# unum-cloud/usearch

Measured on AMD Instinct MI355X. Metric: QPS at recall@10>=0.95, 10000000x768 f16 cos, batch=10000, higher is better.
Workload: dtype f16

## Files before the change

usearch_amd/csrc/engine.hip:

```cpp
#include "engine.hpp"

#include <algorithm>
#include <atomic>
#include <chrono>
#include <cstdio>
#include <cstdlib>
#include <cstring>
#include <thread>

#include <hipcub/hipcub.hpp>

#include "casts.hpp"
#include "host_util.hpp"
#include "kernels.hpp"
#include "search_plan.hpp"

namespace usearch_amd {

static hipError_t scratch_malloc(void** out, std::size_t bytes) {
#ifdef USEARCH_AMD_EXPERIMENT_SCRATCH_MEMORY
    const std::size_t kind = env_size("USEARCH_AMD_SCRATCH_MEMORY", 0);
    if (kind == 1 || kind == 2) {
        const hipError_t e = hipExtMallocWithFlags(out, bytes, kind == 1 ? hipDeviceMallocUncached : hipDeviceMallocFinegrained);
        if (e == hipSuccess)
// ... 870 lines not shown
        ++call.passes;
        UA_HIP(hipStreamSynchronize(stream));
    }
    return nullptr;
}

const char* snapshot_t::search_finish(search_call_t& call, search_stats_t* stats) {
    if (stats)
        *stats = search_stats_t{};
    if (!call.workspace)
        return nullptr;
    struct hand_back_t {
        snapshot_t& owner;
        search_call_t& call;
        ~hand_back_t() {
            if (!call.keep_workspace)
                owner.give_back(call.workspace);
            call.workspace = nullptr;
        }
    } hand_back{*this, call};
    workspace_t& ws = *call.workspace;
    hipStream_t stream = call.stream;
    UA_HIP(hipSetDevice(device_));
    if (call.done) {
        UA_HIP(hipStreamSynchronize(stream));
        return nullptr;
    }

    const std::uint32_t first_grid = call.params.grid, first_lds = call.params.lds_bytes;
    const int first_mode = call.params.mode;
    for (int rung = 0;; ++rung) {
        UA_HIP(hipMemcpyAsync(ws.h_status, ws.d_queue, 24, hipMemcpyDeviceToHost, stream));
        UA_HIP(hipStreamSynchronize(stream));
        if (call.args.sketch_counters) {
            std::uint64_t counters[2];
            std::memcpy(counters, ws.h_status + 2, 16);
            call.plan.stats.sketch_tested += counters[0], call.plan.stats.sketch_pruned += counters[1];
        }
        if (call.params.mode == scratch_global_k) {
            if (ws.h_status[1])
                return "Search scratch overflow in the global-memory pass";
            break;
        }
        if (!ws.h_status[1])
            break;
        UA_HIP(hipMemcpyAsync(ws.h_status + 16, ws.d_status, call.count * 4, hipMemcpyDeviceToHost, stream));
        UA_HIP(hipStreamSynchronize(stream));
        std::vector<std::uint32_t> again;
        if (call.have_todo) {
            for (std::uint32_t q : call.todo)
                if (ws.h_status[16 + q] == status_overflow_k)
                    again.push_back(q);
        } else {
            for (std::uint32_t q = 0; q < call.count; ++q)
                if (ws.h_status[16 + q] == status_overflow_k)
                    again.push_back(q);
        }
        call.todo.swap(again);
        call.have_todo = true;
        call.reran = true;
        if (call.todo.empty())
            break;
        if (rung == 0)
            call.plan.stats.retried_lds = (std::uint32_t)call.todo.size();
        escalate(call.shape, call.knobs, call.plan, rung);
        if (call.plan.mode != scratch_global_k)
            UA_HIP(hipMemcpyAsync(ws.d_todo, call.todo.data(), call.todo.size() * 4, hipMemcpyHostToDevice, stream));
        if (const char* e = run_ladder(call))
            return e;
    }

    if (call.want_phases) {
        unsigned long long ticks[16] = {0};
        UA_HIP(hipMemcpy(ticks, call.args.phases, 128, hipMemcpyDeviceToHost));
        double total = 0;
        for (int i = 0; i < 6; ++i)
            total += (double)ticks[i];
        std::fprintf(stderr, "[usearch_amd] phases ef=%u grid=%u: setup %.1f%% pop+list %.1f%% visited %.1f%% distances %.1f%% "
                             "commit %.1f%% [heap push %.1f%% top insert %.1f%%, %llu candidates rechecked] dump %.1f%% (%.3g ticks); "
                             "frontier pushes %llu, lists ready ahead %llu\n",
                     call.plan.ef, first_grid, 100 * ticks[0] / total, 100 * ticks[1] / total, 100 * ticks[2] / total,
                     100 * ticks[3] / total, 100 * ticks[4] / total, 100 * ticks[8] / total, 100 * ticks[9] / total, ticks[10],
                     100 * ticks[5] / total, total, ticks[6], ticks[7]);
        if (ticks[15])
            std::fprintf(stderr, "[usearch_amd] a team's helpers: %llu hops, ticks measuring per hop %.0f %.0f %.0f %.0f\n", ticks[15],
                         (double)ticks[11] / (double)ticks[15], (double)ticks[12] / (double)ticks[15],
                         (double)ticks[13] / (double)ticks[15], (double)ticks[14] / (double)ticks[15]);
    }
    if (call.want_clock && ws.d_wave_clock && first_grid) {
        std::vector<unsigned long long> clock((std::size_t)first_grid * 2);
        UA_HIP(hipMemcpy(clock.data(), ws.d_wave_clock, clock.size() * 8, hipMemcpyDeviceToHost));
        unsigned long long first = ~0ull, last = 0;
        for (std::uint32_t w = 0; w < first_grid; ++w)
            first = std::min(first, clock[2 * w]), last = std::max(last, clock[2 * w + 1]);
        double gone = 0;
        for (std::uint32_t w = 0; w < first_grid; ++w)
            gone += (double)(clock[2 * w] - first) + (double)(last - clock[2 * w + 1]);
        const double span = (double)(last - first);
        call.plan.stats.tail_idle = span > 0 ? (float)(gone / (span * first_grid)) : 0.f;
        call.plan.stats.span_ms = (float)(span / 1e5);
        if (env_size("USEARCH_AMD_WAVE_CLOCK", 0) > 1) {
            unsigned long long bins[10] = {0};
            for (std::uint32_t w = 0; w < first_grid; ++w)
                ++bins[std::min<std::size_t>(9, (std::size_t)(10.0 * (double)(clock[2 * w + 1] - first) / std::max(span, 1.0)))];
            std::fprintf(stderr, "[usearch_amd] wave exits by tenth of the %.3f ms span (grid %u):", call.plan.stats.span_ms, first_grid);
            for (unsigned long long b : bins)
                std::fprintf(stderr, " %llu", b);
            std::fprintf(stderr, "; idle share %.4f\n", call.plan.stats.tail_idle);
        }
    }
    call.plan.stats.passes = call.passes;
    call.plan.stats.kernel_ms = call.total_ms;
    call.plan.stats.mode = (std::uint32_t)first_mode + 1;
    call.plan.stats.grid = first_grid;
    call.plan.stats.lds_bytes = first_lds;
    if (stats)
        *stats = call.plan.stats;
    if (call.sketch_auto && call.count >= 1024)
        judge_sketch(call.plan.stats.sketch_tested, call.plan.stats.sketch_pruned);
    return nullptr;
}

const char* snapshot_t::search_device(const void* queries, std::size_t count, std::size_t stride_bytes,
                                      std::size_t wanted, std::size_t expansion, std::uint64_t* keys,
                                      float* distances, std::uint64_t* counts, std::uint64_t* visited,
                                      std::uint64_t* computed, hipStream_t stream, const search_tuning_t& tuning,
                                      search_stats_t* stats, bool timed, const search_extras_t* extras) {
    if (stats)
        *stats = search_stats_t{};
    search_call_t call;
    const char* error = search_begin(call, queries, count, stride_bytes, wanted, expansion, keys, distances, counts, visited,
                                     computed, stream, tuning, timed, extras);
    if (error) {
        if (call.workspace)
            give_back(call.workspace);
        return error;
    }
    return search_finish(call, stats);
}

const char* snapshot_t::tune(const void* queries, std::size_t count, std::size_t stride_bytes, std::size_t wanted, std::size_t expansion,
                             std::uint32_t max_trials, std::uint32_t* trials_made) {
    if (trials_made)
        *trials_made = 0;
    max_trials = std::min<std::uint32_t>(max_trials, (std::uint32_t)placement_max_draws_k);
    if (!count || !wanted || !max_trials || !d_vectors_)
        return nullptr;
    UA_HIP(hipSetDevice(device_));
    struct block_t {
        void* p = nullptr;
        ~block_t() { (void)hipFree(p); }
    } results;
    const std::size_t pad = 256, keys_bytes = (count * wanted * 8 + pad - 1) / pad * pad, distances_bytes = (count * wanted * 4 + pad - 1) / pad * pad,
                      column = (count * 8 + pad - 1) / pad * pad;
    UA_HIP(hipMalloc(&results.p, keys_bytes + distances_bytes + 3 * column));
    std::uint8_t* base = static_cast<std::uint8_t*>(results.p);
    const std::uint32_t before = placement_.draws;
    {
        std::lock_guard<std::mutex> lock(pool_mutex_);
        tuning_trials_ = max_trials;
        placement_trials_left_ = max_trials, placement_losses_ = 0, placement_reopens_ = 2;
    }
    const char* failure = nullptr;
    for (std::uint32_t launch = 0; launch < max_trials + 1u && !failure; ++launch) {
        failure = search_device(queries, count, stride_bytes, wanted, expansion, reinterpret_cast<std::uint64_t*>(base),
                                reinterpret_cast<float*>(base + keys_bytes), reinterpret_cast<std::uint64_t*>(base + keys_bytes + distances_bytes),
// ... 436 lines not shown
```

usearch_amd/csrc/kernels.hpp:

```cpp
#pragma once
#include <type_traits>
#include <hip/hip_runtime.h>

#include "common.hpp"
#include "sketch.hpp"

namespace usearch_amd {

#define UA_DEVICE __device__ __forceinline__


UA_DEVICE std::uint32_t lane_id() { return threadIdx.x & 63u; }

template <bool global_ak> UA_DEVICE void wave_sync() {
    if constexpr (global_ak) {
        __builtin_amdgcn_fence(__ATOMIC_RELEASE, "workgroup");
        __builtin_amdgcn_wave_barrier();
        __builtin_amdgcn_fence(__ATOMIC_ACQUIRE, "workgroup");
    } else {
        __builtin_amdgcn_fence(__ATOMIC_RELEASE, "workgroup", "local");
        __builtin_amdgcn_wave_barrier();
        __builtin_amdgcn_fence(__ATOMIC_ACQUIRE, "workgroup", "local");
    }
}
// ... 949 lines not shown
    return chunks * ((scalar_ak == scalar_f16_k || scalar_ak == scalar_bf16_k) ? 32u : 16u);
}

struct team_t {
    std::uint32_t count;
    std::uint32_t leader_in;
    std::uint32_t reserved[2];
    query_norm_t a2;
};
static_assert(sizeof(team_t) <= 64, "the engine reserves 64 bytes for the control block");
constexpr std::uint32_t team_exit_k = 0xFFFFFFFFu;
constexpr std::uint32_t team_ahead_rows_k = 32;
constexpr std::uint32_t team_block_bytes_k = 64 + team_ahead_rows_k * 4;
UA_DEVICE std::uint32_t* team_ahead_list(team_t* team) {
    return reinterpret_cast<std::uint32_t*>(reinterpret_cast<std::uint8_t*>(team) + 64);
}

struct team_landing_t {
    std::uint32_t cell[3] = {0, 0, 0};
};
UA_DEVICE void team_touch_rows(const snapshot_view_t& ix, const std::uint32_t* ahead, std::uint32_t helper, team_landing_t& landing) {
    const std::uint32_t lane = lane_id();
    const std::uint32_t row = helper * 8 + (lane >> 3);
    const std::uint32_t slot = row < team_ahead_rows_k ? ahead[row] : none_slot_k;
    const std::uint32_t halves = (ix.bytes_per_vector + 63u) / 64u;
    const std::uint8_t* half = ix.vectors + (std::uint64_t)slot * ix.row_stride + (lane & 7u) * 64u;
    if (slot != none_slot_k && (lane & 7u) < halves)
        asm volatile("global_load_dword %0, %1, off" : "=&v"(landing.cell[0]) : "v"(half) : "memory");
    if (slot != none_slot_k && 8u + (lane & 7u) < halves)
        asm volatile("global_load_dword %0, %1, off" : "=&v"(landing.cell[1]) : "v"(half + 512) : "memory");
    if (slot != none_slot_k && 16u + (lane & 7u) < halves)
        asm volatile("global_load_dword %0, %1, off" : "=&v"(landing.cell[2]) : "v"(half + 1024) : "memory");
}
UA_DEVICE void team_landing_alive(const team_landing_t& landing) {
    asm volatile("" ::"v"(landing.cell[0]), "v"(landing.cell[1]), "v"(landing.cell[2]));
}

constexpr int team_waves_k = 5;

UA_DEVICE void team_barrier() { asm volatile("s_waitcnt lgkmcnt(0)\n\ts_barrier" ::: "memory"); }

template <int metric_ak, int scalar_ak, int lanes_ak, int loads_ak>
UA_DEVICE void team_share(const snapshot_view_t& ix, const std::uint8_t* query_lds, query_norm_t a2, const std::uint32_t* slots,
                          float* out, std::uint32_t count, std::uint32_t part, std::uint32_t parts, bool in_turn = false) {
    const std::uint32_t per_part = in_turn ? 64u / lanes_ak : (count + parts - 1) / parts;
    const std::uint32_t begin = part * per_part;
    const std::uint32_t end = (in_turn && part + 1 == parts) || begin + per_part > count ? count : begin + per_part;
    if (begin < end)
        measure_rows<metric_ak, scalar_ak, lanes_ak, loads_ak, false, 1>(ix, query_lds, a2, slots + begin, out + begin, end - begin);
}

template <int metric_ak, int scalar_ak, int lanes_ak, int unroll_ak, int mode_ak, int epl_ak, int frontier_ak, int team_ak = 1,
          bool plain_ak = false>
UA_DEVICE bool search_one(const snapshot_view_t& ix, const search_args_t& args, std::uint32_t q,
                          std::uint8_t* query_lds, std::uint8_t* heaps, std::uint32_t* visits, team_t* team = nullptr) {
    constexpr bool global_ak = mode_ak == scratch_global_k;
    constexpr bool in_top_ak = frontier_ak == frontier_top_k;
    static_assert(!in_top_ak || (epl_ak > 0 && !global_ak), "the frontier rides in the register layout of `top`");
    static_assert(!plain_ak || (lanes_ak <= 2 && mode_ak == scratch_hash_k && team_ak == 1 && !in_top_ak), "short rows over the global hash");
    using mem = scratch_gt<global_ak>;
    const std::uint32_t lane = lane_id();
    const std::uint32_t ef = args.ef, wanted = args.wanted;
    const scratch_layout_t layout = scratch_layout(epl_ak ? 0 : ef, in_top_ak ? 0 : args.next_cap, 0);
    top_gt<epl_ak, global_ak, in_top_ak> top;
    top.reset(reinterpret_cast<cand_t*>(heaps + layout.top));
    cand_t* next = reinterpret_cast<cand_t*>(heaps + layout.next);
    std::uint32_t* cand_slots = reinterpret_cast<std::uint32_t*>(heaps + layout.cand_slots);
    float* cand_distances = reinterpret_cast<float*>(heaps + layout.cand_distances);
    const std::uint32_t visits_mask = global_ak ? 0u : args.hash_cap - 1;
    const std::uint32_t visits_limit = global_ak ? 0xFFFFFFFFu : args.hash_cap - args.hash_cap / 4;

#ifdef USEARCH_AMD_PHASES
    std::uint64_t phase_mark = args.phases ? __builtin_amdgcn_s_memtime() : 0;
    std::uint64_t phase_ticks[6] = {0, 0, 0, 0, 0, 0};
    std::uint32_t diagnostic_pushes = 0, diagnostic_ready = 0, diagnostic_rechecks = 0;
    std::uint64_t diagnostic_push_ticks = 0, diagnostic_insert_ticks = 0;
    auto tick = [&](int phase) {
        if (args.phases) {
            const std::uint64_t now = __builtin_amdgcn_s_memtime();
            phase_ticks[phase] += now - phase_mark;
            phase_mark = now;
        }
    };
#else
    auto tick = [](int) {};
#endif
    const std::uint64_t query_row = !plain_ak && args.query_ids ? args.query_ids[q] : q;
    const query_norm_t a2 = stage_query<metric_ak, scalar_ak, lanes_ak>(
        ix, args.queries + query_row * args.query_stride, query_lds);

    if constexpr (!global_ak) {
        uint4* cells = reinterpret_cast<uint4*>(visits);
        const uint4 empty = {none_slot_k, none_slot_k, none_slot_k, none_slot_k};
        for (std::uint32_t i = lane; i < args.hash_cap / 4; i += 64)
            cells[i] = empty;
#ifdef USEARCH_AMD_EXPERIMENT_NO_SLAB_CLEAR_WAIT
        wave_sync<false>();
#else
        if constexpr (mode_ak == scratch_hash_k)
            wave_sync<true>();
        else
            wave_sync<false>();
#endif
    }

    constexpr bool seen_ak = lanes_ak <= 2 && mode_ak == scratch_hash_k && team_ak == 1;
#ifdef USEARCH_AMD_EXPERIMENT_NO_ASIDE
    constexpr bool aside_ak = false;
#else
    constexpr bool aside_ak = plain_ak && lanes_ak == 2;
#endif
    std::uint32_t* seen = nullptr;
    std::uint32_t seen_mask = 0;
    std::uint32_t* aside = nullptr;
    std::uint32_t aside_mask = 0, aside_count = 0;
    if constexpr (aside_ak) {
        aside = reinterpret_cast<std::uint32_t*>(query_lds + args.aside_offset);
        aside_mask = args.aside_cells - 1;
        for (std::uint32_t i = lane; i < args.aside_cells; i += 64)
            aside[i] = none_slot_k;
        wave_sync<false>();
    }
    if constexpr (seen_ak) {
        if (args.seen_cells) {
            seen = reinterpret_cast<std::uint32_t*>(query_lds + args.seen_offset);
            seen_mask = args.seen_cells - 1;
            for (std::uint32_t i = lane; i < args.seen_cells; i += 64)
                seen[i] = none_slot_k;
            wave_sync<false>();
        }
        if (!plain_ak && args.probe_mode == probe_plain_k) {
            std::uint32_t* claim = reinterpret_cast<std::uint32_t*>(query_lds + args.claim_offset);
            for (std::uint32_t i = lane; i < args.claim_bits / 32; i += 64)
                claim[i] = 0u;
            wave_sync<false>();
        }
    }

    constexpr bool sketch_ak = metric_ak == metric_cos_k && f32_math<scalar_ak>() && lanes_ak == 8 && team_ak == 1 && !global_ak && !plain_ak &&
                               unroll_ak % 100 == 12;
    bool sketch_on = false;
    float sketch_margin = 0.f;
    std::uint32_t sketch_tested = 0, sketch_pruned = 0;
    if constexpr (sketch_ak) {
        if (ix.sketch && args.sketch_counters) {
            const float* a = reinterpret_cast<const float*>(query_lds);
            const float* column = ix.sketch_directions + lane;
            float sums[4] = {0.f, 0.f, 0.f, 0.f};
            std::uint32_t i = 0;
            for (; i + 16 <= ix.dimensions; i += 16) {
                float d[16];
#pragma unroll
                for (int u = 0; u < 16; ++u)
                    d[u] = column[(std::size_t)(i + u) * sketch_columns_k];
#pragma unroll
                for (int u = 0; u < 16; ++u)
                    sums[u & 3] = __builtin_fmaf(a[i + u], d[u], sums[u & 3]);
            }
            for (; i < ix.dimensions; ++i)
                sums[0] = __builtin_fmaf(a[i], column[(std::size_t)i * sketch_columns_k], sums[0]);
            const float projected = (sums[0] + sums[1]) + (sums[2] + sums[3]);
            sketch_on = uniform_u32(sketch_norm_in_range((double)a2.f) ? 1u : 0u) != 0u;
            reinterpret_cast<float*>(query_lds + args.sketch_offset)[lane] = sketch_on ? projected / __builtin_sqrtf(a2.f) : 0.f;
            sketch_margin = sketch_slack(ix.dimensions);
            wave_sync<false>();
        }
    }

    std::uint32_t computed = 0, cycles = 0;
    constexpr int loads_ak = unroll_ak % 100, rows_ak = unroll_ak / 100 + 1;
    auto measure = [&](std::uint32_t count) {
        measure_rows<metric_ak, scalar_ak, lanes_ak, loads_ak, global_ak, 1>(ix, query_lds, a2, cand_slots, cand_distances,
                                                                            count);
        computed += count;
    };
    auto measure_hop = [&](std::uint32_t count, float radius_now) {
        if constexpr (sketch_ak) {
            if (sketch_on && top.size == ef) {
                const std::uint32_t sub = lane & 7u, group = lane >> 3;
                const float* coefficients = reinterpret_cast<const float*>(query_lds + args.sketch_offset) + sub * 8;
                const float4 q0 = *reinterpret_cast<const float4*>(coefficients), q1 = *reinterpret_cast<const float4*>(coefficients + 4);
                const std::uint32_t my_slot = lane < count ? mem::load(cand_slots + lane) : 0u;
                for (std::uint32_t base = 0; base < count; base += 32) {
                    uint4 record[4];
#pragma unroll
                    for (int r = 0; r < 4; ++r) {
                        const std::uint32_t ci = base + (std::uint32_t)r * 8 + group;
                        record[r] = uint4{0u, 0u, 0u, 0u};
                        if (ci < count)
                            record[r] = *reinterpret_cast<const uint4*>(ix.sketch + (std::uint64_t)mem::load(cand_slots + ci) * sketch_record_bytes_k + sub * 16);
                    }
#pragma unroll
                    for (int r = 0; r < 4; ++r) {
                        const std::uint32_t ci = base + (std::uint32_t)r * 8 + group;
                        const uint4 v = record[r];
                        const std::uint32_t last = sub == 7u ? 0u : v.w;
                        float dot = 0.f;
                        dot = __builtin_fmaf(half_bits_to_float(v.x & 0xFFFFu), q0.x, dot);
                        dot = __builtin_fmaf(half_bits_to_float(v.x >> 16), q0.y, dot);
                        dot = __builtin_fmaf(half_bits_to_float(v.y & 0xFFFFu), q0.z, dot);
                        dot = __builtin_fmaf(half_bits_to_float(v.y >> 16), q0.w, dot);
                        dot = __builtin_fmaf(half_bits_to_float(v.z & 0xFFFFu), q1.x, dot);
                        dot = __builtin_fmaf(half_bits_to_float(v.z >> 16), q1.y, dot);
                        dot = __builtin_fmaf(half_bits_to_float(last & 0xFFFFu), q1.z, dot);
                        dot = __builtin_fmaf(half_bits_to_float(last >> 16), q1.w, dot);
                        float residual = sub == 7u ? __builtin_bit_cast(float, v.w) : 0.f;
#pragma unroll
                        for (int offset = 1; offset < 8; offset <<= 1) {
                            dot += xor_lane(dot, offset);
                            residual += xor_lane(residual, offset);
                        }
                        if (sub == 0u && ci < count)
                            mem::store(cand_distances + ci, sketch_lower_bound(dot, residual, sketch_margin));
                    }
                }
                wave_sync<false>();
                const float bound = lane < count ? mem::load(cand_distances + lane) : 0.f;
                const std::uint64_t survivors = ballot(lane < count && !(bound >= radius_now));
                const std::uint32_t kept = popcount64(survivors);
                sketch_tested += count, sketch_pruned += count - kept;
                if (kept < count) {
                    const bool survivor = lane_bit(survivors);
                    const std::uint32_t rank = rank_below(survivors, lane);
                    wave_sync<false>();
                    if (survivor)
                        mem::store(cand_slots + rank, my_slot);
                    wave_sync<false>();
                    if (kept)
                        measure_rows<metric_ak, scalar_ak, lanes_ak, loads_ak, global_ak, rows_ak>(ix, query_lds, a2, cand_slots, cand_distances, kept);
                    const float mine = survivor ? mem::load(cand_distances + rank) : bound;
                    wave_sync<false>();
                    if (lane < count) {
                        mem::store(cand_slots + lane, my_slot);
                        mem::store(cand_distances + lane, mine);
                    }
                    wave_sync<false>();
                    computed += count;
                    return;
                }
            }
        }
        if constexpr (team_ak > 1) {
            if (lane == 0)
                team->count = count, team->leader_in = 1u, team->a2 = a2;
            team_barrier();
            team_share<metric_ak, scalar_ak, lanes_ak, loads_ak>(ix, query_lds, a2, cand_slots, cand_distances, count, 0, 4);
            team_barrier();
        } else {
            measure_rows<metric_ak, scalar_ak, lanes_ak, loads_ak, global_ak, rows_ak>(ix, query_lds, a2, cand_slots,
                                                                                       cand_distances, count);
        }
        computed += count;
    };
    auto allowed = [&](std::uint32_t slot) -> bool {
        if constexpr (plain_ak)
            return true;
        if (!ix.has_tombstones && !args.allow_bits && !args.exclude_own)
            return true;
        bool ok = !(args.exclude_own && slot == (std::uint32_t)query_row);
        if (ok && ix.has_tombstones)
            ok = ix.keys[slot] != free_key_k;
        if (ok && args.allow_bits) {
            const std::uint32_t word = slot >> 5, bit = 1u << (slot & 31);
            if (args.known_bits && !(args.known_bits[word] & bit)) {
                ok = slot * 0x9E3779B1u <= args.guess_threshold;
                if (lane == 0) {
                    const std::uint32_t at = atomicAdd(args.ask_cursor, 1u);
                    if (at < args.ask_cap)
                        args.ask_slots[at] = slot, args.ask_keys[at] = ix.keys[slot];
                }
            } else {
                ok = (args.allow_bits[word] & bit) != 0;
            }
        }
        return uniform_u32(ok ? 1u : 0u) != 0;
    };

    std::uint32_t closest = ix.entry_slot;
    if (lane == 0)
        mem::store(cand_slots, closest);
    wave_sync<global_ak>();
    measure(1);
    float closest_distance = uniform_f32(mem::load(cand_distances));
    const std::uint32_t beam_level = plain_ak ? 0u : args.beam_level;
    for (std::uint32_t level = ix.max_level; level > beam_level; --level) {
        bool changed;
        do {
            changed = false;
            const std::uint32_t* list = ix.upper + (std::uint64_t)(ix.upper_ref[closest] + (level - 1)) * ix.m;
            for (std::uint32_t tile = 0; tile < ix.m; tile += 64) {
                const std::uint32_t cell = tile + lane;
                const std::uint32_t neighbor = cell < ix.m ? list[cell] : none_slot_k;
                const std::uint32_t count = popcount64(ballot(neighbor != none_slot_k));
                if (!count)
                    break;
                if (lane < count)
                    mem::store(cand_slots + lane, neighbor);
                wave_sync<global_ak>();
                measure(count);
                const float mine = lane < count ? mem::load(cand_distances + lane) : __builtin_inff();
                float best = mine;
#pragma unroll
                for (int offset = 32; offset >= 1; offset >>= 1)
                    best = fminf(best, __shfl_xor(best, offset, 64));
                if (best < closest_distance) {
                    const std::uint32_t winner =
                        (std::uint32_t)__ffsll((long long)ballot(lane < count && mine == best)) - 1;
                    closest_distance = best;
                    closest = read_lane_u32(neighbor, winner);
                    changed = true;
                }
                wave_sync<global_ak>();
            }
            ++cycles;
        } while (changed);
    }

    std::uint32_t next_size = 0, visits_count = 0, peak_next = 1;
    bool overflow = false;
    if (lane == 0)
        mem::store(cand_slots, closest);
    wave_sync<global_ak>();
    measure(1);
    float radius = uniform_f32(mem::load(cand_distances));
// ... 174 lines not shown
                }
                tick(3);
            }
        }
    }
    for (; !pipelined;) {
        std::uint32_t expanded;
        if constexpr (in_top_ak) {
            float open_distance;
            std::uint32_t owner_lane, owner_cell;
            if (!top.first_open(open_distance, expanded, owner_lane, owner_cell))
                break;
            top.close(owner_lane, owner_cell);
        } else {
            if (!next_size)
                break;
            const cand_t candidate = mem::load(next);
            const float candidate_distance = -uniform_f32(cand_distance(candidate));
            if (candidate_distance > radius && top.size == ef)
                break;
            expanded = uniform_u32(cand_slot(candidate));
        }
        ++cycles;
        const std::uint32_t* list = list_of(expanded);
        const bool list_ready = expanded == ahead_slot;
#ifdef USEARCH_AMD_PHASES
        diagnostic_ready += list_ready ? 1u : 0u;
#endif
        const std::uint32_t ready_cell = ahead_cell;
        std::uint32_t first_cell = none_slot_k;
        if (!list_ready && lane < cells)
            first_cell = list[lane];
        uint4 inline_row = {0u, 0u, 0u, 0u};
        if constexpr (inline_ak) {
            if (inline_rows) {
                if (list_ready)
                    inline_row = ahead_row;
                else if (lane < cells)
                    inline_row = reinterpret_cast<const uint4*>(ix.nbr0_rows)[(std::uint64_t)expanded * cells + lane];
            }
        }
        bool popped = false;
        auto pop_now = [&]() {
            popped = true;
            ahead_slot = none_slot_k;
            if constexpr (in_top_ak) {
                float ahead_distance;
                std::uint32_t ahead_lane, ahead_index;
                if (!top.first_open(ahead_distance, ahead_slot, ahead_lane, ahead_index))
                    ahead_slot = none_slot_k;
            } else {
                heap_pop<global_ak>(next, next_size);
                if (next_size)
                    ahead_slot = uniform_u32(cand_slot(mem::load(next)));
            }
            if (ahead_slot != none_slot_k) {
                ahead_cell = lane < cells ? list_of(ahead_slot)[lane] : none_slot_k;
                if constexpr (inline_ak)
                    if (inline_rows && lane < cells)
                        ahead_row = reinterpret_cast<const uint4*>(ix.nbr0_rows)[(std::uint64_t)ahead_slot * cells + lane];
            }
        };
        if (in_top_ak || !list_ready || cells > 64 || mode_ak == scratch_global_k)
            pop_now();
        for (std::uint32_t tile = 0; tile < cells; tile += 64) {
            const std::uint32_t cell = tile + lane;
            const std::uint32_t neighbor =
                tile == 0 ? (list_ready ? ready_cell : first_cell) : (cell < cells ? list[cell] : none_slot_k);
            const bool present = neighbor != none_slot_k;
            const std::uint32_t present_count = popcount64(ballot(present));
            if (!present_count)
                break;
            if (visits_count + present_count > visits_limit ||
                (!in_top_ak && next_size - (popped ? 0u : 1u) + present_count > args.next_cap)) {
                overflow = true;
                break;
            }
            tick(1);
            bool fresh;
            float early_mine = 0.f;
            bool early_done = false;
            std::uint64_t asked_mask = 0;
            bool measured_early = false;
            if constexpr (mode_ak == scratch_global_k) {
                fresh = visits_set<mode_ak>(visits, visits_mask, neighbor, present);
            } else {
                std::uint32_t h = hash_slot(neighbor) & visits_mask;
                std::uint32_t old = neighbor;
                bool asks = present;
                std::uint32_t seen_cell = 0;
                if constexpr (seen_ak) {
                    if (seen) {
                        seen_cell = ((neighbor * 0x9E3779B1u) >> 9) & seen_mask;
                        asks = present && seen[seen_cell] != neighbor;
                    }
                }
                bool shadow_done = false;
                auto shadow_work = [&]() {
                    if (shadow_done)
                        return;
                    shadow_done = true;
                if constexpr (inline_ak) {
                    if (inline_rows) {
                        partial_t p;
                        accumulate_chunk<metric_ak, scalar_ak>(p, query_lds, 0, inline_row);
                        early_mine = finalize_distance<metric_ak, scalar_ak>(p, a2, ix.dimensions);
                        early_done = true;
                    }
                }
                if constexpr (early_ak) {
                    if (early_rows && tile == 0) {
                        asked_mask = ballot(asks);
                        const std::uint32_t asked = popcount64(asked_mask);
                        if (asks)
                            cand_slots[rank_below(asked_mask, lane)] = neighbor;
                        wave_sync<false>();
                        if (asked)
                            measure_rows<metric_ak, scalar_ak, lanes_ak, loads_ak, false, 1>(ix, query_lds, a2, cand_slots, cand_distances, asked);
                        measured_early = true;
                    }
                }
                };
                std::uint32_t probe_mode = probe_swap_k;
#ifdef USEARCH_AMD_EXPERIMENT_PROBE_MODES
                if constexpr (seen_ak)
                    probe_mode = args.probe_mode;
#endif
                const bool load_first = probe_mode == probe_load_first_k;
                if (probe_mode == probe_plain_k) {
                    std::uint32_t* claim = reinterpret_cast<std::uint32_t*>(query_lds + args.claim_offset);
                    const std::uint32_t claim_mask = args.claim_bits - 1;
                    bool looking = asks;
                    for (;;) {
                        std::uint32_t cell_value = none_slot_k;
                        if (looking)
                            cell_value = __hip_atomic_load(visits + h, __ATOMIC_RELAXED, __HIP_MEMORY_SCOPE_AGENT);
                        if (!popped)
                            pop_now();
                        shadow_work();
                        const bool wants = looking && cell_value == none_slot_k;
                        if (looking && cell_value == neighbor)
                            looking = false;
                        if (ballot(wants)) {
                            const std::uint32_t bit = h & claim_mask;
                            bool won = false;
                            if (wants) {
                                const std::uint32_t before = __hip_atomic_fetch_or(claim + (bit >> 5), 1u << (bit & 31u), __ATOMIC_RELAXED,
                                                                                   __HIP_MEMORY_SCOPE_WORKGROUP);
                                won = ((before >> (bit & 31u)) & 1u) == 0u;
                                claim[bit >> 5] = 0u;
                            }
                            if (won) {
                                __hip_atomic_store(visits + h, neighbor, __ATOMIC_RELAXED, __HIP_MEMORY_SCOPE_AGENT);
                                old = none_slot_k, looking = false;
                            }
                        }
                        if (looking && !wants)
                            h = (h + 1) & visits_mask;
                        if (!ballot(looking))
                            break;
                    }
                } else {
                if (asks) {
                    if (load_first) {
                        old = __hip_atomic_load(visits + h, __ATOMIC_RELAXED, __HIP_MEMORY_SCOPE_AGENT);
                        if (old == none_slot_k)
                            old = atomicCAS(visits + h, none_slot_k, neighbor);
                    } else {
                        old = atomicCAS(visits + h, none_slot_k, neighbor);
                    }
                }
                if (!popped)
                    pop_now();
                shadow_work();
                if constexpr (aside_ak) {
                    bool taken = asks && old != none_slot_k && old != neighbor;
                    const std::uint64_t taken_mask = ballot(taken);
                    if (taken_mask) {
                        if (aside_count + popcount64(taken_mask) > aside_mask - aside_mask / 4) {
                            overflow = true;
                            break;
                        }
                        std::uint32_t cell = ((neighbor * 0x9E3779B1u) >> 11) & aside_mask;
                        do {
                            std::uint32_t there = neighbor;
                            if (taken)
                                there = atomicCAS(aside + cell, none_slot_k, neighbor);
                            if (taken && (there == none_slot_k || there == neighbor))
                                old = there, taken = false;
                            cell = (cell + 1) & aside_mask;
                        } while (ballot(taken));
                        aside_count += popcount64(ballot(lane_bit(taken_mask) && old == none_slot_k));
                    }
                }
                while (!aside_ak && old != none_slot_k && old != neighbor) {
                    h = (h + 1) & visits_mask;
                    if (load_first) {
                        old = __hip_atomic_load(visits + h, __ATOMIC_RELAXED, __HIP_MEMORY_SCOPE_AGENT);
                        if (old == none_slot_k)
                            old = atomicCAS(visits + h, none_slot_k, neighbor);
                    } else {
                        old = atomicCAS(visits + h, none_slot_k, neighbor);
                    }
                }
                }
                fresh = present && old == none_slot_k;
                if constexpr (seen_ak) {
                    if (seen && asks)
                        seen[seen_cell] = neighbor;
                }
            }
            const std::uint64_t fresh_mask = ballot(fresh);
            tick(2);
            const std::uint32_t count = popcount64(fresh_mask);
            visits_count += count;
            if (!count)
                continue;
            float mine = 0.f;
            std::uint32_t mine_slot = 0u;
            bool candidate;
            if (inline_rows) {
                if constexpr (inline_ak) {
                    if (early_done) {
                        mine = early_mine;
                    } else {
                        partial_t p;
                        accumulate_chunk<metric_ak, scalar_ak>(p, query_lds, 0, inline_row);
                        mine = finalize_distance<metric_ak, scalar_ak>(p, a2, ix.dimensions);
                    }
                }
                mine_slot = neighbor;
                candidate = fresh;
                computed += count;
            } else if (measured_early) {
                mine = fresh ? cand_distances[rank_below(asked_mask, lane)] : 0.f;
                mine_slot = neighbor;
                candidate = fresh;
                computed += count;
                wave_sync<false>();
            } else {
                if (fresh)
                    mem::store(cand_slots + rank_below(fresh_mask, lane), neighbor);
                wave_sync<global_ak>();
                measure_hop(count, radius);
                mine = lane < count ? mem::load(cand_distances + lane) : 0.f;
                mine_slot = lane < count ? mem::load(cand_slots + lane) : 0u;
                candidate = lane < count;
            }
            tick(3);

            std::uint64_t pending = ballot(candidate && (top.size < ef || mine < radius));
            while (pending) {
                const std::uint32_t i = (std::uint32_t)__ffsll((long long)pending) - 1;
                pending &= pending - 1;
                const float d = read_lane_f32(mine, i);
#ifdef USEARCH_AMD_PHASES
                ++diagnostic_rechecks;
#endif
                if (!(top.size < ef || d < radius))
                    continue;
                const std::uint32_t successor = read_lane_u32(mine_slot, i);
#ifdef USEARCH_AMD_PHASES
                ++diagnostic_pushes;
                const std::uint64_t t0 = __builtin_amdgcn_s_memtime();
#endif
                push_ticket_t ticket;
                if constexpr (!in_top_ak)
                    ticket = heap_push_begin<global_ak>(next, next_size);
#ifdef USEARCH_AMD_PHASES
                const std::uint64_t t1 = __builtin_amdgcn_s_memtime();
#endif
                if (in_top_ak || allowed(successor))
                    top.insert(d, successor, ef, radius);
                if constexpr (!in_top_ak)
                    heap_push_finish<global_ak>(next, next_size, ticket, -d, successor);
#ifdef USEARCH_AMD_PHASES
                const std::uint64_t t2 = __builtin_amdgcn_s_memtime();
                diagnostic_push_ticks += t1 - t0, diagnostic_insert_ticks += t2 - t1;
#endif
            }
            peak_next = next_size > peak_next ? next_size : peak_next;
            wave_sync<global_ak>();
            tick(4);
        }
        if (overflow)
            break;
        if (!popped)
            pop_now();
    }

    if (overflow) {
        if (lane == 0) {
            args.status[q] = status_overflow_k;
            atomicAdd(args.queue + 1, 1u);
        }
        return false;
    }
    const std::uint32_t found = top.size < wanted ? top.size : wanted;
    top.dump(ix, args, q, found, wanted);
    tick(5);
#ifdef USEARCH_AMD_PHASES
    if (args.phases && lane == 0) {
#pragma unroll
        for (int phase = 0; phase < 6; ++phase)
            atomicAdd(args.phases + phase, (unsigned long long)phase_ticks[phase]);
        atomicAdd(args.phases + 6, (unsigned long long)diagnostic_pushes);
        atomicAdd(args.phases + 7, (unsigned long long)diagnostic_ready);
        atomicAdd(args.phases + 8, (unsigned long long)diagnostic_push_ticks);
        atomicAdd(args.phases + 9, (unsigned long long)diagnostic_insert_ticks);
        atomicAdd(args.phases + 10, (unsigned long long)diagnostic_rechecks);
    }
#endif
    if constexpr (sketch_ak) {
        if (sketch_tested && lane == 0) {
            atomicAdd(args.sketch_counters, (unsigned long long)sketch_tested);
            atomicAdd(args.sketch_counters + 1, (unsigned long long)sketch_pruned);
        }
    }
    if (lane == 0) {
        args.counts[q] = found;
        args.visited[q] = cycles;
        args.computed[q] = computed;
        args.status[q] = status_done_k;
        if (args.peaks) {
            args.peaks[2 * (std::uint64_t)q] = peak_next;
            args.peaks[2 * (std::uint64_t)q + 1] = visits_count;
        }
    }
    return true;
}

enum kernel_variant_t : int {
    variant_u4_w4_k = 0,
    variant_u8_w3_k = 1,
    variant_u12_w2_k = 2,
    variant_u12x2_w2_k = 3,
    variant_count_k = 4,
};
#ifndef USEARCH_AMD_TINY_ROW_WAVES
#define USEARCH_AMD_TINY_ROW_WAVES 6
#endif
#ifndef USEARCH_AMD_SHORT_ROW_WAVES
#define USEARCH_AMD_SHORT_ROW_WAVES 5
#endif
#ifndef USEARCH_AMD_PLAIN_TINY_ROW_WAVES
#define USEARCH_AMD_PLAIN_TINY_ROW_WAVES USEARCH_AMD_TINY_ROW_WAVES
#endif
constexpr int variant_unroll(int v) { return v == variant_u4_w4_k ? 4 : v == variant_u8_w3_k ? 8 : 12; }
constexpr int variant_rows(int v) { return v == variant_u12x2_w2_k ? 2 : 1; }
constexpr int kernel_waves(int variant, int epl, int frontier = 0, int lanes = 8, bool plain = false) {
    if (variant == variant_u12x2_w2_k)
        return 2;
    if (plain && variant == variant_u4_w4_k && epl == 1 && lanes == 1)
        return USEARCH_AMD_PLAIN_TINY_ROW_WAVES;
    if (variant == variant_u4_w4_k && epl == 1 && lanes <= 2)
        return lanes == 1 ? USEARCH_AMD_TINY_ROW_WAVES : USEARCH_AMD_SHORT_ROW_WAVES;
    if (variant == variant_u4_w4_k && epl == 2 && lanes <= 2)
        return USEARCH_AMD_SHORT_ROW_WAVES;
    if (frontier)
        return variant == variant_u4_w4_k ? 4 : variant == variant_u8_w3_k ? 3 : 2;
    return variant == variant_u4_w4_k ? (epl >= 8 ? 3 : 4) : variant == variant_u8_w3_k ? (epl >= 16 ? 2 : 3) : 2;
}

template <int metric_ak, int scalar_ak, int lanes_ak, int variant_ak, int mode_ak, int epl_ak, int frontier_ak, bool plain_ak = false>
__global__ __launch_bounds__(64, kernel_waves(variant_ak, epl_ak, frontier_ak, lanes_ak, plain_ak)) void search_kernel(const snapshot_view_t ix,
                                                                                            const search_args_t args) {
    constexpr int unroll_ak = variant_unroll(variant_ak) + 100 * (variant_rows(variant_ak) - 1);
    extern __shared__ __attribute__((aligned(16))) std::uint8_t lds[];
    std::uint8_t* query_lds = lds;
    const std::uint32_t query_bytes = query_lds_bytes<scalar_ak>(ix.chunks);
    std::uint8_t* slab = args.scratch + (std::uint64_t)blockIdx.x * args.scratch_stride;
    const scratch_layout_t layout = scratch_layout(epl_ak ? 0 : args.ef, frontier_ak == frontier_top_k ? 0 : args.next_cap, 0);
    if (args.wave_clock && lane_id() == 0)
        args.wave_clock[2 * (std::uint64_t)blockIdx.x] = __builtin_amdgcn_s_memrealtime();

    if constexpr (mode_ak == scratch_global_k) {
        const std::uint32_t q = args.todo ? args.todo[blockIdx.x] : blockIdx.x;
        search_one<metric_ak, scalar_ak, lanes_ak, unroll_ak, mode_ak, epl_ak, frontier_ak>(
            ix, args, q, query_lds, slab, reinterpret_cast<std::uint32_t*>(slab + layout.visits));
    } else {
        std::uint8_t* heaps = lds + query_bytes;
        std::uint32_t* visits = mode_ak == scratch_lds_k ? reinterpret_cast<std::uint32_t*>(heaps + layout.visits)
                                                         : reinterpret_cast<std::uint32_t*>(slab);
        for (;;) {
            std::uint32_t ticket = 0;
            if (lane_id() == 0)
                ticket = atomicAdd(args.queue, 1u);
            ticket = uniform_u32(ticket);
            if (ticket >= args.count)
                break;
            const std::uint32_t q = args.todo ? args.todo[ticket] : ticket;
            search_one<metric_ak, scalar_ak, lanes_ak, unroll_ak, mode_ak, epl_ak, frontier_ak, 1, plain_ak>(ix, args, q, query_lds, heaps,
                                                                                                             visits);
// ... 175 lines not shown
```

Baseline: 359,300.

## Prefetch sketch records during visit phase and restructure sketch-pruned hop measurement

Moves the sketch lower-bound filtering out of measure_hop into the main hop loop. When the hop has at most 32 cells, each lane's sketch record is gathered with ds_bpermute and loaded early, during the visited-set insertion, so its latency overlaps with pop and shadow work. Survivors are now always compacted and measured, and small survivor counts use the single-row measure_rows variant to avoid multi-row overhead. It also adds phase diagnostics for sketch bound ticks, at the cost of extra registers for the early records and record loads wasted on candidates that turn out to be already visited.

```diff
diff --git a/usearch_amd/csrc/engine.hip b/usearch_amd/csrc/engine.hip
--- a/usearch_amd/csrc/engine.hip
+++ b/usearch_amd/csrc/engine.hip
@@ -976,6 +976,10 @@
                      call.plan.ef, first_grid, 100 * ticks[0] / total, 100 * ticks[1] / total, 100 * ticks[2] / total,
                      100 * ticks[3] / total, 100 * ticks[4] / total, 100 * ticks[8] / total, 100 * ticks[9] / total, ticks[10],
                      100 * ticks[5] / total, total, ticks[6], ticks[7]);
+        if (!ticks[15] && ticks[12])
+            std::fprintf(stderr, "[usearch_amd] sketch hops %llu: records+bounds %.1f%%, rest of phase 3 (rows; hops before `top` is full included) %.1f%% (of all ticks), hops with more than 8 "
+                                 "survivors %llu\n",
+                         ticks[12], 100 * ticks[11] / total, 100 * ((double)ticks[3] - (double)ticks[11]) / total, ticks[13]);
         if (ticks[15])
             std::fprintf(stderr, "[usearch_amd] a team's helpers: %llu hops, ticks measuring per hop %.0f %.0f %.0f %.0f\n", ticks[15],
                          (double)ticks[11] / (double)ticks[15], (double)ticks[12] / (double)ticks[15],
diff --git a/usearch_amd/csrc/kernels.hpp b/usearch_amd/csrc/kernels.hpp
--- a/usearch_amd/csrc/kernels.hpp
+++ b/usearch_amd/csrc/kernels.hpp
@@ -1055,8 +1055,18 @@
             phase_mark = now;
         }
     };
+    std::uint64_t diagnostic_bound_ticks = 0;
+    std::uint32_t diagnostic_sketch_hops = 0, diagnostic_wide_hops = 0;
+    auto tick_bounds = [&](std::uint32_t kept) {
+        if (args.phases) {
+            diagnostic_bound_ticks += __builtin_amdgcn_s_memtime() - phase_mark;
+            ++diagnostic_sketch_hops;
+            diagnostic_wide_hops += kept > 64u / lanes_ak ? 1u : 0u;
+        }
+    };
 #else
     auto tick = [](int) {};
+    auto tick_bounds = [](std::uint32_t) {};
 #endif
     const std::uint64_t query_row = !plain_ak && args.query_ids ? args.query_ids[q] : q;
     const query_norm_t a2 = stage_query<metric_ak, scalar_ak, lanes_ak>(
@@ -1147,72 +1157,35 @@
                                                                             count);
         computed += count;
     };
-    auto measure_hop = [&](std::uint32_t count, float radius_now) {
-        if constexpr (sketch_ak) {
-            if (sketch_on && top.size == ef) {
-                const std::uint32_t sub = lane & 7u, group = lane >> 3;
-                const float* coefficients = reinterpret_cast<const float*>(query_lds + args.sketch_offset) + sub * 8;
-                const float4 q0 = *reinterpret_cast<const float4*>(coefficients), q1 = *reinterpret_cast<const float4*>(coefficients + 4);
-                const std::uint32_t my_slot = lane < count ? mem::load(cand_slots + lane) : 0u;
-                for (std::uint32_t base = 0; base < count; base += 32) {
-                    uint4 record[4];
-#pragma unroll
-                    for (int r = 0; r < 4; ++r) {
-                        const std::uint32_t ci = base + (std::uint32_t)r * 8 + group;
-                        record[r] = uint4{0u, 0u, 0u, 0u};
-                        if (ci < count)
-                            record[r] = *reinterpret_cast<const uint4*>(ix.sketch + (std::uint64_t)mem::load(cand_slots + ci) * sketch_record_bytes_k + sub * 16);
-                    }
-#pragma unroll
-                    for (int r = 0; r < 4; ++r) {
-                        const std::uint32_t ci = base + (std::uint32_t)r * 8 + group;
-                        const uint4 v = record[r];
-                        const std::uint32_t last = sub == 7u ? 0u : v.w;
-                        float dot = 0.f;
-                        dot = __builtin_fmaf(half_bits_to_float(v.x & 0xFFFFu), q0.x, dot);
-                        dot = __builtin_fmaf(half_bits_to_float(v.x >> 16), q0.y, dot);
-                        dot = __builtin_fmaf(half_bits_to_float(v.y & 0xFFFFu), q0.z, dot);
-                        dot = __builtin_fmaf(half_bits_to_float(v.y >> 16), q0.w, dot);
-                        dot = __builtin_fmaf(half_bits_to_float(v.z & 0xFFFFu), q1.x, dot);
-                        dot = __builtin_fmaf(half_bits_to_float(v.z >> 16), q1.y, dot);
-                        dot = __builtin_fmaf(half_bits_to_float(last & 0xFFFFu), q1.z, dot);
-                        dot = __builtin_fmaf(half_bits_to_float(last >> 16), q1.w, dot);
-                        float residual = sub == 7u ? __builtin_bit_cast(float, v.w) : 0.f;
-#pragma unroll
-                        for (int offset = 1; offset < 8; offset <<= 1) {
-                            dot += xor_lane(dot, offset);
-                            residual += xor_lane(residual, offset);
-                        }
-                        if (sub == 0u && ci < count)
-                            mem::store(cand_distances + ci, sketch_lower_bound(dot, residual, sketch_margin));
-                    }
-                }
-                wave_sync<false>();
-                const float bound = lane < count ? mem::load(cand_distances + lane) : 0.f;
-                const std::uint64_t survivors = ballot(lane < count && !(bound >= radius_now));
-                const std::uint32_t kept = popcount64(survivors);
-                sketch_tested += count, sketch_pruned += count - kept;
-                if (kept < count) {
-                    const bool survivor = lane_bit(survivors);
-                    const std::uint32_t rank = rank_below(survivors, lane);
-                    wave_sync<false>();
-                    if (survivor)
-                        mem::store(cand_slots + rank, my_slot);
-                    wave_sync<false>();
-                    if (kept)
-                        measure_rows<metric_ak, scalar_ak, lanes_ak, loads_ak, global_ak, rows_ak>(ix, query_lds, a2, cand_slots, cand_distances, kept);
-                    const float mine = survivor ? mem::load(cand_distances + rank) : bound;
-                    wave_sync<false>();
-                    if (lane < count) {
-                        mem::store(cand_slots + lane, my_slot);
-                        mem::store(cand_distances + lane, mine);
-                    }
-                    wave_sync<false>();
-                    computed += count;
-                    return;
-                }
-            }
-        }
+    auto record_bound = [&](const uint4 v, const float4 q0, const float4 q1, std::uint32_t sub) -> float {
+        const std::uint32_t last = sub == 7u ? 0u : v.w;
+        float dot = 0.f;
+        dot = __builtin_fmaf(half_bits_to_float(v.x & 0xFFFFu), q0.x, dot);
+        dot = __builtin_fmaf(half_bits_to_float(v.x >> 16), q0.y, dot);
+        dot = __builtin_fmaf(half_bits_to_float(v.y & 0xFFFFu), q0.z, dot);
+        dot = __builtin_fmaf(half_bits_to_float(v.y >> 16), q0.w, dot);
+        dot = __builtin_fmaf(half_bits_to_float(v.z & 0xFFFFu), q1.x, dot);
+        dot = __builtin_fmaf(half_bits_to_float(v.z >> 16), q1.y, dot);
+        dot = __builtin_fmaf(half_bits_to_float(last & 0xFFFFu), q1.z, dot);
+        dot = __builtin_fmaf(half_bits_to_float(last >> 16), q1.w, dot);
+        float residual = sub == 7u ? __builtin_bit_cast(float, v.w) : 0.f;
+#pragma unroll
+        for (int offset = 1; offset < 8; offset <<= 1) {
+            dot += xor_lane(dot, offset);
+            residual += xor_lane(residual, offset);
+        }
+        return sketch_lower_bound(dot, residual, sketch_margin);
+    };
+    auto measure_survivors = [&](std::uint32_t kept) {
+        if constexpr (rows_ak > 1 && narrow_float<scalar_ak>()) {
+            if (kept <= 64u / lanes_ak) {
+                measure_rows<metric_ak, scalar_ak, lanes_ak, loads_ak, global_ak, 1>(ix, query_lds, a2, cand_slots, cand_distances, kept);
+                return;
+            }
+        }
+        measure_rows<metric_ak, scalar_ak, lanes_ak, loads_ak, global_ak, rows_ak>(ix, query_lds, a2, cand_slots, cand_distances, kept);
+    };
+    auto measure_hop = [&](std::uint32_t count) {
         if constexpr (team_ak > 1) {
             if (lane == 0)
                 team->count = count, team->leader_in = 1u, team->a2 = a2;
@@ -1553,6 +1526,8 @@
             bool early_done = false;
             std::uint64_t asked_mask = 0;
             bool measured_early = false;
+            bool records_early = false;
+            uint4 early_record[4];
             if constexpr (mode_ak == scratch_global_k) {
                 fresh = visits_set<mode_ak>(visits, visits_mask, neighbor, present);
             } else {
@@ -1641,6 +1616,20 @@
                         old = atomicCAS(visits + h, none_slot_k, neighbor);
                     }
                 }
+                if constexpr (sketch_ak) {
+                    if (sketch_on && top.size == ef && tile == 0 && cells <= 32) {
+                        records_early = true;
+                        const std::uint32_t present_slot = present ? neighbor : 0u;
+                        std::uint32_t lane_now = lane;
+                        asm volatile("" : "+v"(lane_now));
+                        const int from = (int)((lane_now >> 3) << 2);
+#pragma unroll
+                        for (int r = 0; r < 4; ++r) {
+                            const std::uint32_t slot = (std::uint32_t)__builtin_amdgcn_ds_bpermute(from + r * 32, (int)present_slot);
+                            early_record[r] = *reinterpret_cast<const uint4*>(ix.sketch + ((std::uint64_t)slot * sketch_record_bytes_k + (lane_now & 7u) * 16));
+                        }
+                    }
+                }
                 if (!popped)
                     pop_now();
                 shadow_work();
@@ -1709,11 +1698,75 @@
                 candidate = fresh;
                 computed += count;
                 wave_sync<false>();
+            } else if (sketch_ak && sketch_on && top.size == ef) {
+                const std::uint32_t sub = lane & 7u, group = lane >> 3;
+                bool member;
+                float bound;
+                if (records_early) {
+                    const float* coefficients = reinterpret_cast<const float*>(query_lds + args.sketch_offset) + sub * 8;
+                    const float4 q0 = *reinterpret_cast<const float4*>(coefficients), q1 = *reinterpret_cast<const float4*>(coefficients + 4);
+#pragma unroll
+                    for (int r = 0; r < 4; ++r) {
+                        if (!((fresh_mask >> (r * 8)) & 0xFFu))
+                            continue;
+                        const float lower = record_bound(early_record[r], q0, q1, sub);
+                        if (sub == 0u)
+                            cand_distances[(std::uint32_t)r * 8 + group] = lower;
+                    }
+                    wave_sync<false>();
+                    member = fresh;
+                    mine_slot = neighbor;
+                    bound = fresh ? cand_distances[lane] : 0.f;
+                } else {
+                    if (fresh)
+                        cand_slots[rank_below(fresh_mask, lane)] = neighbor;
+                    wave_sync<false>();
+                    member = lane < count;
+                    mine_slot = member ? cand_slots[lane] : 0u;
+                    const float* coefficients = reinterpret_cast<const float*>(query_lds + args.sketch_offset) + sub * 8;
+                    const float4 q0 = *reinterpret_cast<const float4*>(coefficients), q1 = *reinterpret_cast<const float4*>(coefficients + 4);
+                    for (std::uint32_t base = 0; base < count; base += 32) {
+                        uint4 record[4];
+#pragma unroll
+                        for (int r = 0; r < 4; ++r) {
+                            const std::uint32_t ci = base + (std::uint32_t)r * 8 + group;
+                            record[r] = uint4{0u, 0u, 0u, 0u};
+                            if (ci < count)
+                                record[r] = *reinterpret_cast<const uint4*>(ix.sketch + (std::uint64_t)cand_slots[ci] * sketch_record_bytes_k + sub * 16);
+                        }
+#pragma unroll
+                        for (int r = 0; r < 4; ++r) {
+                            if (base + (std::uint32_t)r * 8 >= count)
+                                break;
+                            const std::uint32_t ci = base + (std::uint32_t)r * 8 + group;
+                            const float lower = record_bound(record[r], q0, q1, sub);
+                            if (sub == 0u && ci < count)
+                                cand_distances[ci] = lower;
+                        }
+                    }
+                    wave_sync<false>();
+                    bound = member ? cand_distances[lane] : 0.f;
+                }
+                const std::uint64_t survivors = ballot(member && !(bound >= radius));
+                const std::uint32_t kept = popcount64(survivors);
+                sketch_tested += count, sketch_pruned += count - kept;
+                tick_bounds(kept);
+                const bool survivor = lane_bit(survivors);
+                wave_sync<false>();
+                if (survivor)
+                    cand_slots[rank_below(survivors, lane)] = mine_slot;
+                wave_sync<false>();
+                if (kept)
+                    measure_survivors(kept);
+                mine = survivor ? cand_distances[rank_below(survivors, lane)] : bound;
+                candidate = member;
+                computed += count;
+                wave_sync<false>();
             } else {
                 if (fresh)
                     mem::store(cand_slots + rank_below(fresh_mask, lane), neighbor);
                 wave_sync<global_ak>();
-                measure_hop(count, radius);
+                measure_hop(count);
                 mine = lane < count ? mem::load(cand_distances + lane) : 0.f;
                 mine_slot = lane < count ? mem::load(cand_slots + lane) : 0u;
                 candidate = lane < count;
@@ -1780,6 +1833,11 @@
         atomicAdd(args.phases + 8, (unsigned long long)diagnostic_push_ticks);
         atomicAdd(args.phases + 9, (unsigned long long)diagnostic_insert_ticks);
         atomicAdd(args.phases + 10, (unsigned long long)diagnostic_rechecks);
+        if constexpr (team_ak == 1) {
+            atomicAdd(args.phases + 11, (unsigned long long)diagnostic_bound_ticks);
+            atomicAdd(args.phases + 12, (unsigned long long)diagnostic_sketch_hops);
+            atomicAdd(args.phases + 13, (unsigned long long)diagnostic_wide_hops);
+        }
     }
 #endif
     if constexpr (sketch_ak) {
```

After: 421,700 (median of 6 runs). 1.17x the previous value.
